# Abhipray/audio-codec

Hardware: AMD Instinct MI355X
Metric: audio channel-frames/s encode (48 kHz, 1024-line long blocks, 128 kb/s/ch) (higher is better)
Workload: dtype f64

## Files before the change

### audio-codec_amd/csrc/k_psy.hip

```cpp
#include "pacx_launch.h"
#include "mdct_dev.h"
#include "pcm_stage.h"
#include "wave_np_sum.h"
#include "quant_dev.h"


template <int DT>
__device__ __forceinline__ double hann_sample(const typename PcmStage<DT>::elem *raw, int i,
                                              const double *__restrict__ hw,
                                              const double *__restrict__ hw_pcm)
{
    if constexpr (DT == 0) {
        const int c = raw[i];
        return hw_pcm[i] * (double)(c == -32768 ? 0 : c);
    } else {
        return hw[i] * raw[i];
    }
}

#ifdef PACX_PSY_DEBUG
__device__ long long g_psy_dbg[16 * 16];
#define PSY_T(k) do { long long t_; asm volatile("s_waitcnt lgkmcnt(0)\n\ts_memtime %0\n\ts_waitcnt lgkmcnt(0)" : "=s"(t_) :: "memory"); \
                      if (dbg_on) dbg_acc[k] += t_ - dbg_last; dbg_last = t_; } while (0)
extern "C" int pacx_debug_read_psy(long long *out, int n)
// ... 526 lines not shown
        const int m = (64 - k) & 63;
        const cplx tm = c_mul(T.w128[m], po);
        cplx zm = c_add(pe, tm), zm5 = c_sub(pe, tm);
        if (k == 0) {
            zm5 = zk;
            zm = zk5;
        }
        ig[k] = pair_intensity(zk, zm5, T.w256[k], T.norm_short);
        ig[k + 64] = pair_intensity(zk5, zm, T.w256[k + 64], T.norm_short);
        if (k == 0)
            ig[128] = pair_intensity(zk, zk, T.w256[128], T.norm_short);
    }
    __syncthreads();

    int count = 0;
    for (int base = 0; base <= 128; base += 8) {
        const int i = base + r;
        bool pk = false;
        if (i >= 1 && i <= 128) {
            const double c = ig[i];
            pk = (c > ig[i - 1]) && (i == 128 || c > ig[i + 1]);
        }
        const unsigned m = (unsigned)((__builtin_amdgcn_ballot_w64(pk) >> (8 * g)) & 0xFFull);
        if (pk)
            pk_idx[g][count + __popc(m & ((1u << r) - 1u))] = (unsigned char)i;
        count += __popc(m);
    }
    if (r == 0) {
        pk_cnt[g] = count;
        n_peaks[cf * PACX_SUB + g] = count;
        n_kept_out[cf * PACX_SUB + g] = count;
    }
    __syncthreads();
    int start[PACX_SUB + 1];
    start[0] = 0;
#pragma unroll
    for (int q = 0; q < PACX_SUB; ++q)
        start[q + 1] = start[q] + pk_cnt[q];
    const int total = start[PACX_SUB];
    for (int t = lane; t < total; t += 64) {
        int q = 0;
#pragma unroll
        for (int u = 1; u < PACX_SUB; ++u)
            q += (t >= start[u]);
        const int p = t - start[q];
        const int i = pk_idx[q][p];
        const double *iq = inten + q * 130;
        peaks[cf * PACX_MAX_PEAKS + q * 64 + p] = make_peak(iq[i - 1], iq[i], i, T.fstep_short);
    }
}

#ifndef MASK_WAVES
#define MASK_WAVES 4
#endif
#ifndef MASK_OCC
#define MASK_OCC 3
#endif
#ifndef MASK_LDS_TABLES
#define MASK_LDS_TABLES 1
#endif
#ifndef MASK_OCC_PLAIN
#define MASK_OCC_PLAIN 4
#endif
#ifndef MASK_WG_PER_CU
#define MASK_WG_PER_CU 3
#endif
#ifndef MASK_WG_PER_CU_PLAIN
#define MASK_WG_PER_CU_PLAIN 4
#endif



__device__ __forceinline__ unsigned long long mask_key_of(double v)
{
    const unsigned long long u = (unsigned long long)__double_as_longlong(v);
    return (u >> 63) ? ~u : (u | 0x8000000000000000ull);
}
__device__ __forceinline__ double mask_value_of(unsigned long long k)
{
    const unsigned long long u = (k >> 63) ? (k & 0x7fffffffffffffffull) : ~k;
    return __longlong_as_double((long long)u);
}

#ifndef MASK_WAVES_PLAIN
#define MASK_WAVES_PLAIN 4
#endif
constexpr int mask_waves(int m, bool tail) { return (m == PACX_M_LONG && !tail) ? MASK_WAVES_PLAIN : MASK_WAVES; }

template <int M, bool TAIL>
__global__ __launch_bounds__(64 * mask_waves(M, TAIL), (M == PACX_M_LONG && !TAIL) ? MASK_OCC_PLAIN : MASK_OCC) void k_mask(PacxTables T, const uint8_t *__restrict__ flags,
                                                         int n_ch, long long n_units, int mixed,
                                                         const PacxPeak *__restrict__ peaks,
                                                         const int32_t *__restrict__ n_peaks,
                                                         const double *__restrict__ lines,
                                                         double *__restrict__ smr,
                                                         double *__restrict__ thr_out,
                                                         const int32_t *__restrict__ cf_list,
                                                         const int32_t *__restrict__ cf_count,
                                                         MaskTail tail)
{
    constexpr bool SHORT = (M == PACX_M_SHORT);
    constexpr int NW = mask_waves(M, TAIL);
    static_assert(!(TAIL && SHORT), "the fused tail is for long blocks");
    constexpr int PER = M / 64;
    constexpr bool BARK_LDS = (MASK_LDS_TABLES & 1) != 0, QUIET_LDS = (MASK_LDS_TABLES & 2) != 0;
    __shared__ __attribute__((aligned(16))) double bark_l[BARK_LDS ? M : 1];
    __shared__ __attribute__((aligned(16))) double quiet_l[QUIET_LDS ? M : 1];
    __shared__ __attribute__((aligned(16))) double chunk_c[PER][4];
    constexpr bool PAD = M / 64 == 16;
    constexpr int RJ = PAD ? PER / 2 : 0;
    constexpr int NH = PAD ? 2 : 1, HP = PER / NH;
    constexpr int MH = M / NH;
    constexpr int JSTR = PAD ? 72 : 64;
    __shared__ __attribute__((aligned(16))) double bufs[NW][MH + (PAD ? MH / 8 : 0)];
    __shared__ __attribute__((aligned(16))) double2 mk_zs_all[NW][64];
    __shared__ __attribute__((aligned(16))) double mk_u_all[NW][64];
    const int tid = threadIdx.x, lane = tid & 63, wv = tid >> 6;
    const double *__restrict__ bark_g = SHORT ? T.bark_short : T.bark_long;
    const double *__restrict__ quiet_g = SHORT ? T.thresh_short : T.thresh_long;
    for (int i = tid; i < M; i += 64 * NW) {
        if (BARK_LDS)
            bark_l[i] = bark_g[i];
        if (QUIET_LDS)
            quiet_l[i] = quiet_g[i];
    }
    __syncthreads();
    const double *bark_s = BARK_LDS ? (const double *)bark_l : bark_g;
    const double *quiet_s = QUIET_LDS ? (const double *)quiet_l : quiet_g;
    for (int j = wv; j < PER; j += NW) {
        double qm = quiet_s[64 * j + lane];
#pragma unroll
        for (int off = 32; off > 0; off >>= 1)
            qm = fmin(qm, __shfl_xor(qm, off, 64));
        if (lane == 0) {
            chunk_c[j][0] = bark_s[64 * j] - 0.5;
            chunk_c[j][1] = bark_s[64 * j + 63] + 0.5;
            chunk_c[j][2] = qm - 0.01;
        }
    }
    __syncthreads();

    double *buf = bufs[wv];
    const int sl = lane + (PAD ? lane >> 3 : 0);
    double2 *mk_zs = mk_zs_all[wv];
    double *mk_u = mk_u_all[wv];
    const int nb = SHORT ? T.nb_short : T.nb_long;
    const int32_t *__restrict__ lower = SHORT ? T.band_lower_short : T.band_lower_long;
    const int32_t *__restrict__ count = SHORT ? T.band_lines_short : T.band_lines_long;
    if (cf_list)
        n_units = SHORT ? (long long)(*cf_count) * PACX_SUB : (long long)(*cf_count);
#ifdef PACX_PSY_DEBUG
    const bool dbg_on = blockIdx.x == 5;
    long long dbg_acc[8] = {0, 0, 0, 0, 0, 0, 0, 0}, dbg_last = 0;
    unsigned long long st_pairs = 0, st_surv = 0, st_live = 0, st_batches = 0;
    PSY_T(7);
    dbg_acc[7] = 0;
#endif
    for (long long unit = (long long)blockIdx.x * NW + wv; unit < n_units;
         unit += (long long)gridDim.x * NW) {
        long long cf = SHORT ? unit / PACX_SUB : unit;
        const int sb = SHORT ? (int)(unit % PACX_SUB) : 0;
        if (cf_list) {
            cf = cf_list[cf];
        } else if (mixed) {
            const unsigned fl = flags ? flags[cf / n_ch] : 0u;
            if (SHORT != ((fl & 2u) != 0))
                continue;
        }
        const PacxPeak *__restrict__ pk = peaks + cf * PACX_MAX_PEAKS + sb * 64;
        const int np = n_peaks[cf * PACX_SUB + sb];
        const long long loff = cf * PACX_M_LONG + sb * PACX_M_SHORT;

        double rb[RJ ? RJ : 1];
#pragma unroll
        for (int j = 0; j < PER; ++j) {
            if (j < RJ)
                rb[j] = -INFINITY;
            else
                buf[sl + JSTR * (j - RJ)] = -INFINITY;
        }
        PacxPeak qn;
        qn.z = 0.0; qn.spl = -1000.0; qn.slope = 0.0;
        if (lane < np)
            qn = pk[lane];
        PSY_T(0);
        for (int pb = 0; pb < np; pb += 64) {
#ifdef PACX_PSY_DEBUG
            st_batches += 1;
#endif
            const PacxPeak q = qn;
            qn.z = 0.0; qn.spl = -1000.0; qn.slope = 0.0;
            if (pb + 64 + lane < np)
                qn = pk[pb + 64 + lane];
            const double lvl = q.spl - 16.0;
            const int n_in = min(64, np - pb);
            const double bz_lo = __hiloint2double(__builtin_amdgcn_readlane(__double2hiint(q.z), 0),
                                                  __builtin_amdgcn_readlane(__double2loint(q.z), 0));
            const double bz_hi = __hiloint2double(__builtin_amdgcn_readlane(__double2hiint(q.z), n_in - 1),
                                                  __builtin_amdgcn_readlane(__double2loint(q.z), n_in - 1));
            const double b_lvl = wave_max_upper(lvl);
            const double b_slope = wave_max_upper(q.slope);
            wave_lds_fence();
            mk_zs[lane] = make_double2(q.z, q.spl);
            mk_u[lane] = q.slope;
            wave_lds_fence();
#pragma unroll
            for (int j = 0; j < PER; ++j) {
                asm volatile("" ::: "memory");
                const double lo_edge = chunk_c[j][0], hi_edge = chunk_c[j][1], need = chunk_c[j][2];
                if (b_slope <= 0.0) {
                    double bb = 0.0;
                    if (bz_hi < lo_edge)
                        bb = b_slope * (lo_edge - bz_hi);
                    else if (bz_lo > hi_edge)
                        bb = -27.0 * (bz_lo - hi_edge);
                    if (b_lvl + bb <= need)
                        continue;
                }
                const double ub = q.slope * fmax(lo_edge - q.z, 0.0) + -27.0 * fmax(q.z - hi_edge, 0.0);
                const bool live = (q.slope > 0.0 && q.spl > -1000.0) || (lvl + ub > need);
                unsigned long long todo = __builtin_amdgcn_ballot_w64(live);
#ifdef PACX_PSY_DEBUG
                st_pairs += 1;
                st_surv += __popcll(todo);
                st_live += todo ? 1 : 0;
#endif
                if (!todo)
                    continue;
                const double zj = bark_s[lane + 64 * j];
                double bj;
                if (j < RJ)
                    bj = rb[j];
                else
                    bj = buf[sl + JSTR * (j - RJ)];
                while (todo) {
                    int bs[4];
#pragma unroll
                    for (int u = 0; u < 4; ++u) {
                        bs[u] = __builtin_ctzll(todo);
                        if (todo & (todo - 1))
                            todo &= todo - 1;
                        else if (u == 3)
                            todo = 0;
                    }
                    double2 zs[4];
                    double pus[4];
#pragma unroll
                    for (int u = 0; u < 4; ++u) {
                        zs[u] = mk_zs[bs[u]];
                        pus[u] = mk_u[bs[u]];
                    }
#pragma unroll
                    for (int u = 0; u < 4; ++u) {
                        const double pz = zs[u].x, ps = zs[u].y, pu = pus[u];
                        const double dz = zj - pz;
                        const double a = fmax(fabs(dz) - 0.5, 0.0);
                        const double gain = (dz < 0.0 ? -27.0 : pu) * a;
                        const double cand = (ps + gain) - 16.0;
                        asm("v_max_f64 %0, %1, %2" : "=v"(bj) : "v"(bj), "v"(cand));
                    }
                }
                if (j < RJ)
                    rb[j] = bj;
                else
                    buf[sl + JSTR * (j - RJ)] = bj;
            }
        }
        wave_lds_fence();
        PSY_T(1);
        double *__restrict__ out = smr ? smr + cf * T.band_stride + sb * T.nb_short : nullptr;
        unsigned long long *key = (unsigned long long *)mk_zs;
        key[lane] = 0ull;
#pragma unroll 1
        for (int h = NH - 1; h >= 0; --h) {
            if (RJ && h == 0) {
                wave_lds_fence();
#pragma unroll
                for (int j = 0; j < RJ; ++j)
                    buf[sl + JSTR * j] = rb[j];
                wave_lds_fence();
            }
            const int k0 = h * MH;
            double v_next = lines[loff + k0 + lane], q_next = quiet_s[k0 + lane];
#pragma unroll 1
            for (int j = 0; j < HP; ++j) {
                const int k = k0 + lane + 64 * j;
                const double v = v_next;
                double thr = q_next;
                if (j + 1 < HP) {
                    v_next = lines[loff + k + 64];
                    q_next = quiet_s[k + 64];
                }
                const double bst = buf[sl + JSTR * j];
                if (bst > -INFINITY)
                    thr = fmax(thr, mask_round_trip(bst));
                if (thr_out)
                    thr_out[loff + k] = thr;
                double it = (v * v) * 4.0;
                if (it == 0.0)
                    it = 1e-8;
                double spl = 96.0 + 10.0 * pacx_log10_pos(it + PACX_EPS);
                if (spl < -30.0)
                    spl = -30.0;
                buf[sl + JSTR * j] = spl - thr;
            }
            wave_lds_fence();
            int rl = lane;
            asm volatile("" : "+v"(rl));
            double v[HP];
            uint8_t bd[HP];
            if constexpr (SHORT) {
                const double2 t = *(const double2 *)(buf + 2 * rl);
                v[0] = t.x;
                v[1] = t.y;
                const uchar2 b2 = *(const uchar2 *)(T.line_band_short + 2 * rl);
                bd[0] = b2.x;
                bd[1] = b2.y;
            } else {
                static_assert(SHORT || HP == 8, "eight lines per lane and half");
                const uint2 b8 = *(const uint2 *)(T.line_band_long + k0 + 8 * rl);
                const unsigned w[2] = {b8.x, b8.y};
#pragma unroll
                for (int j = 0; j < HP; ++j) {
                    v[j] = buf[9 * rl + j];
                    bd[j] = (uint8_t)(w[j >> 2] >> (8 * (j & 3)));
                }
            }
            wave_lds_fence();
            int cur = bd[0];
            double mx = v[0];
#pragma unroll
            for (int j = 1; j < HP; ++j) {
                if (bd[j] != cur) {
                    atomicMax(&key[cur], mask_key_of(mx));
                    cur = bd[j];
                    mx = v[j];
                } else {
                    mx = fmax(mx, v[j]);
                }
            }
            atomicMax(&key[cur], mask_key_of(mx));
        }
        wave_lds_fence();
        PSY_T(2);
        const double s_l = mask_value_of(key[lane & 31]);
        if (out && lane < nb)
            out[lane] = s_l;
        {
            if constexpr (TAIL) {
                wave_lds_fence();
                int tl = lane;
                asm volatile("" : "+v"(tl));
                char *base = (char *)buf;
                unsigned *words = (unsigned *)base;
                double *cp = (double *)(base + PACX_PAYLOAD_STRIDE);
                unsigned long long *bmax = (unsigned long long *)(base + 2704);
                int *ba_s = (int *)(base + 2960), *sf_s = ba_s + PACX_MAX_BANDS;
                int *offs = sf_s + PACX_MAX_BANDS, *lower_s = offs + PACX_MAX_BANDS + 1;
                const int half = tl >> 5, l = tl & 31;
                const unsigned fl = flags ? flags[cf / n_ch] : 0u;
                const long long boff = cf * T.band_stride;
                const int32_t *__restrict__ n_lines = T.use_sbr ? T.band_lines_long_alloc : T.band_lines_long;
                const double budget = pacx_bit_budget(T.target_bps, PACX_M_LONG, 0, (fl & 5u) != 0, T.n_scale_bits,
                                                      T.n_mant_size_bits, nb, T.use_vq, T.use_sbr);
                int max_mant = 1 << T.n_mant_size_bits;
                if (max_mant > 16)
                    max_mant = 16;
                const bool has = half == 0 && l < nb;
                const int nl = has ? n_lines[l] : 0;
                int bits = 0, cap = 0;
                bitalloc_half(half == 0, has, has ? s_l : 0.0, nl, budget, max_mant, cp + 32 * half, half, l, bits, cap, T.guard != 0, T.nb_long);
                if (has) {
                    tail.bit_alloc[boff + l] = bits;
                    ba_s[l] = bits;
                }
                if (tl == nb && nb < PACX_MAX_BANDS)
                    ba_s[nb] = 0;
                if (cap && tail.status && tl == 0)
                    atomicOr(&tail.status[cf], ((cap & 1) ? 4u : 0u) | ((cap & 2) ? 16u : 0u));
                PSY_T(4);
                if (!T.use_vq) {
                    const int ov = tail.overall[cf * PACX_SUB];
                    const int k0 = 16 * tl;
                    int my_off = 0, a_mine = 0, end = 0;
                    if (tail.payload) {
                        for (int i = tl; i < PACX_PAYLOAD_WORDS; i += 64)
                            words[i] = 0u;
                        wave_lds_fence();
                        a_mine = (tl < nb) ? ba_s[tl] : 0;
                        const int width = (tl < nb) ? T.n_mant_size_bits + T.n_scale_bits + a_mine * count[tl] : 0;
                        int incl = width;
#pragma unroll
                        for (int off = 1; off < 32; off <<= 1) {
                            const int t = __shfl_up(incl, off, 64);
                            if (tl >= off)
                                incl += t;
                        }
                        my_off = 3 + T.n_scale_bits + incl - width;
                        end = __shfl(incl, nb - 1, 64) + 3 + T.n_scale_bits;
                        if (tl < nb) {
                            offs[tl] = my_off + T.n_mant_size_bits + T.n_scale_bits;
                            lower_s[tl] = lower[tl];
                        }
                        if (tl == 0) {
                            put_bits(words, 0, fl & 1u, 1);
                            put_bits(words, 1, (fl >> 1) & 1u, 1);
                            put_bits(words, 2, (fl >> 2) & 1u, 1);
                            put_bits(words, 3, (unsigned)ov, T.n_scale_bits);
                        }
                    }
                    double x[16];
                    uint8_t band[16];
                    long_scale_factors(T, lines + loff, (double)(1 << ov), bmax, ba_s, sf_s, tl, x, band);
                    if (tl < nb) {
                        tail.scale_factor[boff + tl] = sf_s[tl];
                        if (tail.payload) {
                            put_bits(words, my_off, (unsigned)(a_mine ? a_mine - 1 : 0), T.n_mant_size_bits);
                            put_bits(words, my_off + T.n_mant_size_bits, (unsigned)sf_s[tl], T.n_scale_bits);
                        }
                    }
                    PSY_T(5);
                    bool near = false;
#pragma unroll
                    for (int j4 = 0; j4 < 16; j4 += 4) {
                        int mq[4];
#pragma unroll
                        for (int u = 0; u < 4; ++u) {
                            const int j = j4 + u;
                            const int b = band[j];
                            const int a = ba_s[b];
                            mq[u] = a ? pacx_mantissa(x[j], sf_s[b], T.n_scale_bits, a) : 0;
                            if (T.guard)
                                near = near || pacx_quant_guard(fabs(x[j]), (1 << T.n_scale_bits) - 1 + a, PACX_GUARD_LINE_ERR);
                            if (tail.payload && a)
                                put_bits(words, offs[b] + (k0 + j - lower_s[b]) * a, (unsigned)mq[u], a);
                        }
                        if (tail.mantissa)
                            *(int4 *)(tail.mantissa + loff + k0 + j4) = make_int4(mq[0], mq[1], mq[2], mq[3]);
                    }
                    if (tail.status && __builtin_amdgcn_ballot_w64(near) && tl == 0)
                        atomicOr(&tail.status[cf], 16u);
                    if (tail.payload) {
                        wave_lds_fence();
                        const int nbytes = ((end - 3) + 4 + 7) >> 3;
                        unsigned *dst = (unsigned *)(tail.payload + cf * (long long)tail.payload_stride);
                        for (int i = tl; i < (nbytes + 3) / 4; i += 64)
                            dst[i] = __builtin_bswap32(words[i]);
                        if (tl == 0)
                            tail.n_bytes[cf] = nbytes;
                    }
                    PSY_T(6);
                }
            }
        }
        wave_lds_fence();
        PSY_T(3);
    }
#ifdef PACX_PSY_DEBUG
    if (dbg_on && lane == 0 && M == PACX_M_LONG)
        for (int k = 0; k < 8; ++k)
            g_psy_dbg[wv * 16 + k] = dbg_acc[k];
    if (lane == 0 && M == PACX_M_LONG) {
        atomicAdd((unsigned long long *)&g_psy_dbg[160], st_pairs);
        atomicAdd((unsigned long long *)&g_psy_dbg[161], st_surv);
        atomicAdd((unsigned long long *)&g_psy_dbg[162], st_live);
        atomicAdd((unsigned long long *)&g_psy_dbg[163], st_batches);
    }
#endif
}

#define SMRG_THREADS 256
__global__ __launch_bounds__(SMRG_THREADS) void k_smr_generic(long long n_blocks, int n, int nb,
                                                             const double *__restrict__ data,
                                                             const double *__restrict__ lines,
                                                             const double *__restrict__ hann,
                                                             const double *__restrict__ tw_cos,
                                                             const double *__restrict__ tw_sin, double norm,
                                                             double fstep, const double *__restrict__ bark,
                                                             const double *__restrict__ quiet,
                                                             const int32_t *__restrict__ band_lower,
                                                             const int32_t *__restrict__ band_count,
                                                             double *__restrict__ smr, double *__restrict__ thr_out,
                                                             int32_t *__restrict__ n_peaks_out)
{
    extern __shared__ __attribute__((aligned(16))) unsigned char smrg_lds[];
    const int half = n / 2, n_bins = half + 1, max_pk = half / 2 + 1;
    double *w = (double *)smrg_lds;
    double *inten = w + n;
    PacxPeak *pk = (PacxPeak *)(inten + n_bins + (n_bins & 1));
    __shared__ int n_pk;
    const int tid = threadIdx.x;
    const long long blk = blockIdx.x;
    if (blk >= n_blocks)
        return;
    const double *x = data + blk * n;
    for (int i = tid; i < n; i += SMRG_THREADS)
        w[i] = hann[i] * x[i];
    if (tid == 0)
        n_pk = 0;
    __syncthreads();
    for (int k = tid; k < n_bins; k += SMRG_THREADS) {
        double re = 0.0, im = 0.0;
        int m = 0;
        for (int i = 0; i < n; ++i) {
            re += w[i] * tw_cos[m];
            im -= w[i] * tw_sin[m];
            m += k;
            if (m >= n)
                m -= n;
        }
        const double a = sqrt(re * re + im * im);
        inten[k] = norm * (a * a);
    }
    __syncthreads();
    for (int i = 1 + tid; i < n_bins; i += SMRG_THREADS) {
        const double c = inten[i];
        if (c > inten[i - 1] && (i == n_bins - 1 || c > inten[i + 1])) {
            const int at = atomicAdd(&n_pk, 1);
            if (at < max_pk)
                pk[at] = make_peak(inten[i - 1], c, i, fstep);
        }
    }
    __syncthreads();
    const int np = n_pk < max_pk ? n_pk : max_pk;
    if (tid == 0 && n_peaks_out)
        n_peaks_out[blk] = np;
    const double *ln = lines + blk * half;
    for (int k = tid; k < half; k += SMRG_THREADS) {
        const double zj = bark[k];
        double best = -INFINITY;
        for (int p = 0; p < np; ++p) {
            const double dz = zj - pk[p].z;
            const double a = fmax(fabs(dz) - 0.5, 0.0);
            const double gain = (dz < 0.0 ? -27.0 : pk[p].slope) * a;
            best = fmax(best, (pk[p].spl + gain) - 16.0);
        }
        double thr = quiet[k];
        if (best > -INFINITY)
            thr = fmax(thr, mask_round_trip(best));
        if (thr_out)
            thr_out[blk * half + k] = thr;
        const double v = ln[k];
        double it = (v * v) * 4.0;
        if (it == 0.0)
            it = 1e-8;
        double spl = 96.0 + 10.0 * pacx_log10_pos(it + PACX_EPS);
        if (spl < -30.0)
            spl = -30.0;
        w[k] = spl - thr;
// ... 109 lines not shown
```

### audio-codec_amd/csrc/pacx_api.hip

```cpp
#include <hip/hip_runtime.h>

#include <math.h>
#include <stdio.h>
#include <stdlib.h>
#include <string.h>

#include <cmath>
#include <string>
#include <vector>

#include "../../include/pacx.h"
#include "body_index.h"
#include "pacx_launch.h"
#include "pvq_dev.h"
#include "pacx_vq_tables.h"
#include "pacx_tables_gen.h"

using namespace pacx_k;

struct PacxOverrides {
    int split_short;
    int fuse_tail;
    int fuse_front;
    int vq_fuse_alloc;
    int vq_frame;
    int vq_bfs;
    int vq_dec_frame;
};

#define PACX_FUSE_FRONT_DEFAULT 1

static int env_override(const char *name, int lo, int hi)
{
    const char *e = getenv(name);
    if (!e || !*e)
        return -1;
    char *end;
    const long v = strtol(e, &end, 10);
    return (*end || v < lo || v > hi) ? -1 : (int)v;
}

static PacxOverrides read_overrides(void)
{
    PacxOverrides o;
    o.split_short = env_override("PACX_SPLIT_SHORT", 0, 0);
    o.fuse_tail = env_override("PACX_FUSE_TAIL", 0, 1);
    o.fuse_front = env_override("PACX_FUSE_FRONT", 0, 1);
    o.vq_fuse_alloc = env_override("PACX_VQ_FUSE_ALLOC", 0, 1);
    o.vq_frame = env_override("PACX_VQ_FRAME", 0, 0);
    o.vq_bfs = env_override("PACX_VQ_BFS", 0, 1 << 20);
    o.vq_dec_frame = env_override("PACX_VQ_DEC_FRAME", 0, 0);
    return o;
}

struct pacx_handle {
    int device;
    int n_cu;
    PacxOverrides force;
    PacxTables T;
    std::vector<void *> owned;
    long long ws_cf;
    double *ws_lines;
    double *ws_smr;
    PacxPeak *ws_peaks;
    int32_t *ws_npeaks;
    int32_t *ws_nkept;
    int32_t *ws_overall;
    long long *ws_chunks;
    long long *ws_offs;
    int32_t *ws_lists;
    long long ws_blocks_cf;
    double *ws_blocks;
    int fork_side;
    hipStream_t side_stream;
    hipEvent_t ev_fork, ev_join;
    hipStream_t short_stream;
    hipStream_t spare_stream;
    hipEvent_t ev_short_done, ev_lists;
    std::vector<char> vq_view;
    std::vector<char> vqdec_view;
    int tables_exact;
    long long ws_mant_cf;
    int32_t *ws_mant;
    long long ws_dec_cf;
    double *ws_dec_lines;
    uint8_t *ws_dec_sbr;
    uint32_t *ws_dec_status;
    double *ws_sbr_mean;
    long long ws_vq_cf;
    unsigned *ws_unit_words;
    int32_t *ws_unit_bits;
    long long ws_index_bytes;
    char *ws_index;
    long long ws_thr_cf;
    double *ws_thr;
    uint32_t *ws_rate_status;
    long long ws_solve_n;
    char *ws_solve;
    long long *ws_seg;
    long long seg_host_n;
    long long *seg_host;
    hipEvent_t ev_seg;
    std::string err;
};

static thread_local std::string g_create_err;

static int fail(pacx_handle *h, int code, const std::string &msg)
{
    if (h)
        h->err = msg;
    else
        g_create_err = msg;
    return code;
}

#define HIP_TRY(h, call)                                                               \
    do {                                                                               \
        hipError_t e_ = (call);                                                        \
        if (e_ != hipSuccess)                                                          \
            return fail(h, PACX_E_HIP, std::string(#call) + ": " + hipGetErrorString(e_)); \
    } while (0)

static void drain_internal(pacx_handle *h);
#define HIP_TRY_FORKED(h, call)                                                        \
    do {                                                                               \
        hipError_t e_ = (call);                                                        \
        if (e_ != hipSuccess) {                                                        \
            drain_internal(h);                                                         \
            return fail(h, PACX_E_HIP, std::string(#call) + ": " + hipGetErrorString(e_)); \
        }                                                                              \
// ... 258 lines not shown
        TRY(upload(h, hsp.data(), hsp.size(), &T.hann_short_pcm));
    }

    {
        std::vector<double2> t;
        t = unit_circle(512, 8, 1, 8192);  TRY(upload(h, t.data(), t.size(), &T.tw_long));
        t = unit_circle(64, 8, 1, 1024);   TRY(upload(h, t.data(), t.size(), &T.tw_short));
        t = unit_circle(512, 2, 0, 512);   TRY(upload(h, t.data(), t.size(), &T.w512));
        t = unit_circle(512, 2, 0, 1024);
        for (int k = 1; k < 256; ++k)
            t[512 - k] = make_double2(-t[k].x, t[k].y);
        t[256].x = 0.0;
        TRY(upload(h, t.data(), t.size(), &T.w1024));
        t = unit_circle(1025, 2, 0, 2048);
        for (int k = 0; k <= 512; ++k)
            t[k + 512] = make_double2(t[k].y, -t[k].x);
        TRY(upload(h, t.data(), t.size(), &T.w2048));
        t = unit_circle(64, 2, 0, 128);    TRY(upload(h, t.data(), t.size(), &T.w128));
        t = unit_circle(129, 2, 0, 256);   TRY(upload(h, t.data(), t.size(), &T.w256));
    }

    {
        std::vector<double> bl(ML), tl(ML), bs(MS), ts(MS);
        const int ri = gen_rate_index(cfg->sample_rate);
        const double *g_bl = ri >= 0 ? (const double *)PACX_GEN_BARK_LONG + (size_t)ri * ML : nullptr;
        const double *g_tl = ri >= 0 ? (const double *)PACX_GEN_THRESH_LONG + (size_t)ri * ML : nullptr;
        const double *g_bs = ri >= 0 ? (const double *)PACX_GEN_BARK_SHORT + (size_t)ri * MS : nullptr;
        const double *g_ts = ri >= 0 ? (const double *)PACX_GEN_THRESH_SHORT + (size_t)ri * MS : nullptr;
        if (ri < 0 && (!cfg->bark_long || !cfg->thresh_long || !cfg->bark_short || !cfg->thresh_short))
            h->tables_exact = 0;
        for (int k = 0; k < ML; ++k) {
            const double f = (sr / (2 * ML)) * (k + 0.5);
            bl[k] = cfg->bark_long ? cfg->bark_long[k] : (g_bl ? g_bl[k] : pacx_bark(f));
            tl[k] = cfg->thresh_long ? cfg->thresh_long[k] : (g_tl ? g_tl[k] : pacx_thresh_quiet(f));
        }
        for (int k = 0; k < MS; ++k) {
            const double f = (sr / (2 * MS)) * (k + 0.5);
            bs[k] = cfg->bark_short ? cfg->bark_short[k] : (g_bs ? g_bs[k] : pacx_bark(f));
            ts[k] = cfg->thresh_short ? cfg->thresh_short[k] : (g_ts ? g_ts[k] : pacx_thresh_quiet(f));
        }
        TRY(upload(h, bl.data(), bl.size(), &T.bark_long));
        TRY(upload(h, tl.data(), tl.size(), &T.thresh_long));
        TRY(upload(h, bs.data(), bs.size(), &T.bark_short));
        TRY(upload(h, ts.data(), ts.size(), &T.thresh_short));
    }
    auto hanning_norm = [](int n) {
        long double acc = 0;
        for (int i = 0; i < n; ++i) {
            const long double w = 0.5L - 0.5L * cosl(2.0L * 3.14159265358979323846264338327950288L * i / (n - 1));
            acc += w * w;
        }
        return (double)(4.0L / ((long double)n * n * (acc / n)));
    };
    (void)hanning_norm;
    T.norm_long = cfg->fft_norm_long != 0.0 ? cfg->fft_norm_long : ((const double *)PACX_GEN_FFT_NORM)[0];
    T.norm_short = cfg->fft_norm_short != 0.0 ? cfg->fft_norm_short : ((const double *)PACX_GEN_FFT_NORM)[1];
    T.fstep_long = cfg->fft_freq_step_long != 0.0 ? cfg->fft_freq_step_long : 1.0 / (NL * (1.0 / sr));
    T.fstep_short = cfg->fft_freq_step_short != 0.0 ? cfg->fft_freq_step_short : 1.0 / (NS * (1.0 / sr));

    {
        std::vector<double> bb(NL / 2 + 1);
        for (int i = 0; i <= NL / 2; ++i)
            bb[i] = pacx_bark((double)i * T.fstep_long);
        TRY(upload(h, bb.data(), bb.size(), &T.bark_bin_long));
    }
    T.nb_long = cfg->n_bands_long;
    T.nb_short = cfg->n_bands_short;
    int covered_long = ML, covered_short = MS;
    TRY(build_bands(h, cfg->band_lines_long, T.nb_long, ML, &T.band_lower_long, &T.band_lines_long,
                    &T.line_band_long, &covered_long));
    TRY(build_bands(h, cfg->band_lines_short, T.nb_short, MS, &T.band_lower_short, &T.band_lines_short,
                    &T.line_band_short, &covered_short));
    if (covered_short < MS && T.nb_short >= 8) {
        g_create_err = "pacx_create: at most 7 short bands when they do not cover every line";
        pacx_destroy(h);
        return PACX_E_UNSUPPORTED;
    }
    T.band_stride = T.nb_long > PACX_SUB * T.nb_short ? T.nb_long : PACX_SUB * T.nb_short;
    T.n_scale_bits = cfg->n_scale_bits;
    T.n_mant_size_bits = cfg->n_mant_size_bits;
    T.target_bps = cfg->target_bits_per_sample;

    T.guard = cfg->guard ? 1 : 0;
    T.use_vq = cfg->use_vq ? 1 : 0;
    T.use_sbr = cfg->use_sbr ? 1 : 0;
    T.first_omitted = T.nb_long;
    T.band_lines_long_alloc = T.band_lines_long;
    if (T.use_sbr) {
        std::vector<int32_t> alloc_lines(cfg->band_lines_long, cfg->band_lines_long + T.nb_long);
        const int cut = (covered_long - 1) / 2;
        int at = 0;
        for (int b = 0; b < T.nb_long; ++b) {
            if (at >= cut) {
                if (T.first_omitted == T.nb_long)
                    T.first_omitted = b;
                alloc_lines[b] = 1;
            }
            at += cfg->band_lines_long[b];
        }
        if (T.nb_long - T.first_omitted > PACX_SUB) {
            g_create_err = "pacx_create: more than 8 SBR-omitted bands";
            pacx_destroy(h);
            return PACX_E_UNSUPPORTED;
        }
        TRY(upload(h, alloc_lines.data(), alloc_lines.size(), &T.band_lines_long_alloc));
    }
    PvqTables tab;
    memset(&tab, 0, sizeof(tab));
    tab.l_max = 1;
    const double *d_lt = nullptr;
    if (T.use_vq) {
        int l_max = 1;
        for (int b = 0; b < T.nb_long; ++b)
            l_max = cfg->band_lines_long[b] > l_max ? cfg->band_lines_long[b] : l_max;
        for (int b = 0; b < T.nb_short; ++b)
            l_max = cfg->band_lines_short[b] > l_max ? cfg->band_lines_short[b] : l_max;
        tab.l_max = l_max;
        PacxVqHostTables vt;
        pacx_vq_build(l_max, cfg->half_log2 ? cfg->half_log2 : (const double *)PACX_GEN_HALF_LOG2, &vt);
        if (vt.n_tab.empty()) {
            vt.n_tab.push_back(0);
            vt.p_tab.push_back(0);
        }
        TRY(upload(h, vt.n_tab.data(), vt.n_tab.size(), &tab.n_tab));
        TRY(upload(h, vt.p_tab.data(), vt.p_tab.size(), &tab.p_tab));
        TRY(upload(h, vt.row_off.data(), vt.row_off.size(), &tab.row_off));
        TRY(upload(h, vt.k_of.data(), vt.k_of.size(), &tab.k_of));
        TRY(upload(h, vt.w_of.data(), vt.w_of.size(), &tab.w_of));
        TRY(upload(h, vt.half_log2.data(), vt.half_log2.size(), &tab.half_log2));
        h->vq_view.resize(pacx_vq_view_size());
        std::vector<int32_t> sizes_long(cfg->band_lines_long, cfg->band_lines_long + T.nb_long);
        for (int b = T.first_omitted; b < T.nb_long; ++b)
            sizes_long[b] = 1;
        std::vector<double> lt((1u << PACX_VQ_THETA_TABLE_BITS) - 1, 0.0);
        memcpy(lt.data(), cfg->vq_log2_tan ? cfg->vq_log2_tan : (const double *)PACX_GEN_VQ_LOG2_TAN,
               sizeof(double) * lt.size());
        static_assert(sizeof(PACX_GEN_VQ_LOG2_TAN) / 8 == (1u << PACX_VQ_THETA_TABLE_BITS) - 1, "log2-tan table");
        TRY(upload(h, lt.data(), lt.size(), &d_lt));
        pacx_vq_view_fill(h->vq_view.data(), tab, cfg->log_mu1 != 0.0 ? cfg->log_mu1 : ((const double *)PACX_GEN_LOG_MU1)[0],
                          d_lt, sizes_long.data(), T.nb_long, cfg->band_lines_short, T.nb_short);
    }
    if (T.use_vq || T.use_sbr) {
        const int gr = cfg->sbr_gauss ? cfg->sbr_gauss_radius : 800;
        if (gr < 1 || gr > 4096) {
            g_create_err = "pacx_create: sbr_gauss_radius out of range";
            pacx_destroy(h);
            return PACX_E_ARG;
        }
        std::vector<double> gw(2 * gr + 1), lf(ML);
        static_assert(sizeof(PACX_GEN_SBR_GAUSS) / 8 == 2 * 800 + 1, "gaussian weights");
        memcpy(gw.data(), cfg->sbr_gauss ? cfg->sbr_gauss : (const double *)PACX_GEN_SBR_GAUSS,
               sizeof(double) * gw.size());
        for (int k = 0; k < ML; ++k)
            lf[k] = cfg->line_freq_long ? cfg->line_freq_long[k] : (k + 0.5) * (sr / (2 * ML));
        const double *d_gw, *d_lf;
        TRY(upload(h, gw.data(), gw.size(), &d_gw));
        TRY(upload(h, lf.data(), lf.size(), &d_lf));
        h->vqdec_view.resize(pacx_vqdec_view_size());
        pacx_vqdec_view_fill(h->vqdec_view.data(), tab, d_lt, d_gw, gr, d_lf, cfg->band_lines_long, T.nb_long,
                             cfg->band_lines_short, T.nb_short);
    }
#undef TRY
    *out = h;
    return PACX_OK;
}

// ... 1408 lines not shown
```

### audio-codec_amd/csrc/pacx_dev.h

```cpp
#ifndef PACX_DEV_H
#define PACX_DEV_H

#include <hip/hip_runtime.h>
#include <stdint.h>

#include "pacx_exact.h"

#define PACX_N_LONG 2048
#define PACX_M_LONG 1024
#define PACX_N_SHORT 256
#define PACX_M_SHORT 128
#define PACX_SUB 8
#define PACX_SHORT_FIRST 448
#define PACX_MAX_PEAKS 512
#define PACX_PAYLOAD_STRIDE 2192
#define PACX_PAYLOAD_WORDS (PACX_PAYLOAD_STRIDE / 4)

struct PacxTables {
    const double *win_long;
    const double *win_short;
    const double *hann_long;
    const double *hann_short;
    const double *ones;
    const double *kbd_long;
    const double *kbd_short;
    const double *hann_long_pcm;
    const double *hann_short_pcm;
    const double2 *tw_long;
    const double2 *tw_short;
    const double2 *w512;
    const double2 *w1024;
    const double2 *w2048;
    const double2 *w128;
    const double2 *w256;
    const double *bark_long, *thresh_long;
    const double *bark_short, *thresh_short;
    const double *bark_bin_long;
    const int32_t *band_lower_long, *band_lines_long;
    const int32_t *band_lower_short, *band_lines_short;
    const uint8_t *line_band_long;
    const uint8_t *line_band_short;
    double norm_long, norm_short;
    double fstep_long, fstep_short;
    double target_bps;
    int nb_long, nb_short;
    int n_scale_bits, n_mant_size_bits;
    int band_stride;
    int use_vq, use_sbr;
    int first_omitted;
    const int32_t *band_lines_long_alloc;
    int guard;
};

struct PacxPcmView {
    const void *base;
    long long frame_stride, ch_stride, samp_stride;
    int n_ch;
};

struct __attribute__((aligned(8))) PacxPeak {
    double z;
    double spl;
    double slope;
};

#define PACX_PART_LONG  (1 << 4)
#define PACX_PART_SHORT (2 << 4)

struct MaskTail {
    const int32_t *overall;
    int32_t *bit_alloc;
    int32_t *scale_factor;
    int32_t *mantissa;
    uint32_t *status;
    uint8_t *payload;
    int32_t *n_bytes;
    int payload_stride;
};

__device__ __forceinline__ unsigned pacx_xcd_block(unsigned b, unsigned n_blocks)
{
    return (n_blocks & 7u) ? b : (b & 7u) * (n_blocks >> 3) + (b >> 3);
}
__device__ __forceinline__ long long pacx_xcd_frame(unsigned b, unsigned n_blocks, long long n_cf)
{
    if ((n_cf & 2047) != 0 || n_blocks != (unsigned)n_cf)
        return b;
    const unsigned idx = b >> 3;
    return (long long)(idx >> 8) * 2048 + (b & 7u) * 256 + (idx & 255u);
}

struct PacxIndexWs {
    long long n_seg, n_groups;
    size_t tab;
    size_t gtab;
    size_t gentry;
    size_t gbase;
    size_t entry;
    size_t base;
    size_t fin;
};

#endif
```

### audio-codec_amd/csrc/pacx_exact.h

```cpp
#ifndef PACX_EXACT_H
#define PACX_EXACT_H

#include <math.h>
#include <stdint.h>
#include <string.h>

#if defined(__HIPCC__)
#define PACX_HD __host__ __device__ __forceinline__
#else
#define PACX_HD static inline
#endif

#define PACX_MAX_BANDS 32
#define PACX_ALLOC_MAX_PASSES 200
#define PACX_DB_PER_BIT 6.2
#define PACX_EPS 2.220446049250313e-16
#define PACX_VQ_SPLIT_BITS 32
#define PACX_VQ_THETA_TABLE_BITS 12

PACX_HD double pacx_pcm16_to_f64(int c)
{
    const int neg = c < 0;
    const int mag = (neg ? -c : c) & 32767;
    const double n = (double)(2 * mag);
// ... 359 lines not shown
    rc = fma(fma(-d, rc, 1.0), rc, rc);
    double sq = f * rc;
    sq = fma(fma(-d, sq, f), rc, sq);
    const double z = sq * sq, w = z * z;
#if defined(__HIP_DEVICE_COMPILE__)
#define PACX_FMA_SC(r, a, b, c) asm("v_fma_f64 %0, %1, %2, %3" : "=v"(r) : "v"(a), "v"(b), "s"(c))
#else
#define PACX_FMA_SC(r, a, b, c) (r) = fma((a), (b), (c))
#endif
    double h1, h2;
    PACX_FMA_SC(h1, w, Lg6, Lg4);
    PACX_FMA_SC(h1, w, h1, Lg2);
    PACX_FMA_SC(h2, w, Lg7, Lg5);
    PACX_FMA_SC(h2, w, h2, Lg3);
    PACX_FMA_SC(h2, w, h2, Lg1);
#undef PACX_FMA_SC
    const double t1 = w * h1;
    const double t2 = z * h2;
    const double r = sq * (hfsq + (t2 + t1));
    double hi = f - hfsq;
    memcpy(&bits, &hi, 8);
    bits &= 0xFFFFFFFF00000000ull;
    memcpy(&hi, &bits, 8);
    const double lo = ((f - hi) - hfsq) + r;
    double val_hi = hi * ivln10hi;
    const double y2 = dk * log10_2hi;
    double val_lo = fma(dk, log10_2lo, fma(lo + hi, ivln10lo, lo * ivln10hi));
    const double wv = y2 + val_hi;
    val_lo += (y2 - wv) + val_hi;
    return val_lo + wv;
}

PACX_HD double pacx_spl_array(double intensity)
{
    if (intensity == 0.0)
        intensity = 1e-8;
    double spl = 96.0 + 10.0 * log10(fabs(intensity) + PACX_EPS);
    if (spl < -30.0)
        spl = -30.0;
    return spl;
}

PACX_HD double pacx_exp2_lean(double y)
{
    const double n = rint(y), f = y - n;
    const double c1 = 6.931471805599453094e-01, c2 = 2.402265069591007123e-01, c3 = 5.550410866482157995e-02,
                 c4 = 9.618129107628477162e-03, c5 = 1.333355814642844343e-03, c6 = 1.540353039338160995e-04,
                 c7 = 1.525273380405984028e-05, c8 = 1.321548679014430949e-06, c9 = 1.017808600923969973e-07,
                 c10 = 7.054911620801123330e-09;
#if defined(__HIP_DEVICE_COMPILE__)
#define PACX_FMA_SC(r, a, b, c) asm("v_fma_f64 %0, %1, %2, %3" : "=v"(r) : "v"(a), "v"(b), "s"(c))
#else
#define PACX_FMA_SC(r, a, b, c) (r) = fma((a), (b), (c))
#endif
    double p;
    PACX_FMA_SC(p, f, c10, c9);
    PACX_FMA_SC(p, f, p, c8);
    PACX_FMA_SC(p, f, p, c7);
    PACX_FMA_SC(p, f, p, c6);
    PACX_FMA_SC(p, f, p, c5);
    PACX_FMA_SC(p, f, p, c4);
    PACX_FMA_SC(p, f, p, c3);
    PACX_FMA_SC(p, f, p, c2);
    PACX_FMA_SC(p, f, p, c1);
#undef PACX_FMA_SC
    p = fma(f, p, 1.0);
    int e = (int)n;
    return ldexp(p, e);
}

PACX_HD double pacx_spl_of_intensity_of(double x)
{
    double y = (96.0 - x) * 0.33219280948873623;
    if (y > 1000.0)
        y = 1000.0;
    const double t = PACX_EPS * pacx_exp2_lean(y);
    if (!(t < 1e-3))
        return -30.0;
    const double p = t * (1.0 + t * (-0.5 + t * (1.0 / 3.0 + t * (-0.25 + t * 0.2))));
    const double r = x + 4.3429448190325182765 * p;
    return r < -30.0 ? -30.0 : r;
}

PACX_HD double pacx_spl_scalar(double intensity)
{
    if (intensity == 0.0)
        return -30.0;
    double spl = 96.0 + 10.0 * log10(fabs(intensity) + PACX_EPS);
    if (spl < -30.0)
        spl = -30.0;
    return spl;
}

PACX_HD double pacx_bark(double f)
{
    const double t = f / 7500.0;
    return 13.0 * atan(0.76 * f / 1000.0) + 3.5 * atan(t * t);
}

PACX_HD double pacx_thresh_quiet(double f)
{
    if (f < 10.0)
        f = 10.0;
    const double k = f / 1000.0;
    const double d = k - 3.3;
    return 3.64 * pow(k, -0.8) - 6.5 * exp(-0.6 * (d * d)) + 0.001 * (k * k * k * k);
}

PACX_HD int pacx_window_kind(unsigned flags)
{
    const int last_t = flags & 1u, cur_t = (flags >> 1) & 1u, next_t = (flags >> 2) & 1u;
    if (cur_t) return 0;
    if (last_t && next_t) return 3;
    if (last_t) return 2;
    if (next_t) return 1;
    return 0;
}

#endif
```

### audio-codec_amd/engine.py

```python
import ctypes

import numpy as np
import torch

from . import _lib, tables
from .psychoac import ScaleFactorBands, AssignMDCTLinesFromFreqLimits

N_LONG, N_SHORT = 1024, 128


def _ptr(t):
    return ctypes.c_void_p(t.data_ptr()) if t is not None else None


class PcmView:

    def __init__(self, tensor, n_channels, n_frames, frame_stride, channel_stride,
                 sample_stride=1):
        if tensor.dtype == torch.int16:
            dt = _lib.PCM_I16
        elif tensor.dtype == torch.float64:
            dt = _lib.PCM_F64
        else:
            raise TypeError("PCM must be int16 codes or float64 signed fractions")
# ... 602 lines not shown
    def _elem(self, name, x, *ints):
        x = x.contiguous()
        out = self._empty(x.shape, torch.int64)
        self._call(name, ctypes.c_int64(x.numel()), _ptr(x), *[int(i) for i in ints], _ptr(out),
                   self._stream())
        return out

    def quantize_uniform(self, x, n_bits):
        return self._elem("pacx_quantize_uniform", x, n_bits)

    def scale_factor(self, x, n_scale_bits, n_mant_bits):
        return self._elem("pacx_scale_factor", x, n_scale_bits, n_mant_bits)

    def mantissa(self, x, scale, n_scale_bits, n_mant_bits):
        return self._elem("pacx_mantissa", x, scale, n_scale_bits, n_mant_bits)

    def mantissa_fp(self, x, scale, n_scale_bits, n_mant_bits):
        return self._elem("pacx_mantissa_fp", x, scale, n_scale_bits, n_mant_bits)

    def _delem(self, name, codes, *ints):
        codes = codes.contiguous()
        assert codes.dtype == torch.int64
        out = self._empty(codes.shape, torch.float64)
        self._call(name, ctypes.c_int64(codes.numel()), _ptr(codes), *[int(i) for i in ints], _ptr(out),
                   self._stream())
        return out

    def dequantize_uniform(self, codes, n_bits):
        return self._delem("pacx_dequantize_uniform", codes, n_bits)

    def dequantize(self, mant, scale, n_scale_bits, n_mant_bits):
        return self._delem("pacx_dequantize", mant, scale, n_scale_bits, n_mant_bits)

    def dequantize_fp(self, mant, scale, n_scale_bits, n_mant_bits):
        return self._delem("pacx_dequantize_fp", mant, scale, n_scale_bits, n_mant_bits)

    def imdct(self, lines, short=False):
        lines = lines.contiguous().view(-1, N_LONG)
        out = self._empty((lines.shape[0], 2 * N_LONG), torch.float64)
        self._call("pacx_imdct_batch", ctypes.c_int64(lines.shape[0]), _lib.MDCT_SHORT if short else 0, _ptr(lines),
                   _ptr(out), self._stream())
        return out

    def mdct_direct(self, x, a, b, inverse=False):
        n_in = (a + b) // 2 if inverse else a + b
        n_out = a + b if inverse else (a + b) // 2
        x = x.contiguous().view(-1, n_in)
        out = self._empty((x.shape[0], n_out), torch.float64)
        self._call("pacx_mdct_direct_batch", ctypes.c_int64(x.shape[0]), int(a), int(b), int(bool(inverse)), _ptr(x),
                   _ptr(out), self._stream())
        return out

    def transient_detect(self, blocks, thresh=4.5):
        blocks = blocks.contiguous()
        n, n_ch, ln = blocks.shape
        out = self._empty((n,), torch.uint8)
        self._call("pacx_transient_detect_f64", ctypes.c_int64(n), int(n_ch), int(ln), _ptr(blocks),
                   ctypes.c_double(float(thresh)), _ptr(out), self._stream())
        return out

    def bit_alloc_generic(self, budget, max_mant_bits, n_lines, smr):
        smr = smr.contiguous()
        n, nb = smr.shape
        nl = torch.as_tensor(np.asarray(n_lines, dtype=np.int32), device=self.device)
        bits = self._empty((n, nb), torch.int32)
        self._call("pacx_bitalloc_generic", ctypes.c_int64(n), int(nb), _ptr(nl), _ptr(budget.contiguous()),
                   int(max_mant_bits), _ptr(smr), _ptr(bits), self._stream())
        return bits


class EncoderPool:

    def __init__(self, n, *args, **kwargs):
        self.encs = [Encoder(*args, **kwargs) for _ in range(max(1, int(n)))]
        dev = self.encs[0].device
        self.streams = [torch.cuda.Stream(device=dev) for _ in self.encs]
        self.done = [torch.cuda.Event() for _ in self.encs]
        self._turn = 0
        self._gate = self._gate_stream = None
        self._used = [False] * len(self.encs)
        if len(self.encs) > 1:
            for e in self.encs:
                e.set_side_fork(True)

    def __len__(self):
        return len(self.encs)

    def next(self):
        k = self._turn
        self._turn = (k + 1) % len(self.encs)
        return k

    def slot(self, k):
        pool = self

        class _Slot:
            def __enter__(self_inner):
                self_inner.ctx = torch.cuda.stream(pool.streams[k])
                self_inner.ctx.__enter__()
                return pool.encs[k]

            def __exit__(self_inner, *exc):
                pool.done[k].record(pool.streams[k])
                pool._used[k] = True
                return self_inner.ctx.__exit__(*exc)
        return _Slot()

    def align(self, delay_us=None):
        if len(self.encs) < 2:
            return
        if delay_us is None:
            delay_us = float(os.environ.get("PACX_POOL_GATE_US", "100"))
        if delay_us <= 0 or not hasattr(torch.cuda, "_sleep"):
            return
        dev = self.encs[0].device
        if self._gate is None:
            self._gate_stream = torch.cuda.Stream(device=dev)
            self._gate = torch.cuda.Event()
            t0, t1 = torch.cuda.Event(enable_timing=True), torch.cuda.Event(enable_timing=True)
            with torch.cuda.stream(self._gate_stream):
                torch.cuda._sleep(100_000)
                t0.record()
                torch.cuda._sleep(2_000_000)
                t1.record()
            t1.synchronize()
            self._cycles_per_us = 2_000_000 / max(t0.elapsed_time(t1) * 1e3, 1.0)
        with torch.cuda.stream(self._gate_stream):
            for k in range(len(self.encs)):
                if self._used[k]:
                    self._gate_stream.wait_event(self.done[k])
            torch.cuda._sleep(int(delay_us * self._cycles_per_us))
            self._gate.record(self._gate_stream)
        for s in self.streams:
            s.wait_event(self._gate)

    def wait(self, k, stream=None):
        (stream or torch.cuda.current_stream(self.encs[0].device)).wait_event(self.done[k])

    def synchronize(self):
        for s in self.streams:
            s.synchronize()

    def close(self):
        for e in self.encs:
            e.close()
```

Before: 52.57 million.

## Screen mask lines with cheap float log before exact per-band SMR max

Adds a screening pass to the long-block mask kernel. It computes an approximate per-line SMR using a float log2 and a lower-bound threshold, takes a per-band approximate max, and keeps only lines within a small delta of that max. Only those candidates, up to 64 per half, are evaluated with the exact double-precision SPL and mask round trip, and it falls back to the full path on overflow. This is meant to avoid the exact per-line log and threshold conversion for most of the 1024 lines, at the cost of extra ballots, LDS atomics and a rigorously bounded approximation window. It also moves the pool gate calibration into the constructor so it is no longer done on the first align call.

```diff
diff --git a/audio-codec_amd/csrc/k_psy.hip b/audio-codec_amd/csrc/k_psy.hip
--- a/audio-codec_amd/csrc/k_psy.hip
+++ b/audio-codec_amd/csrc/k_psy.hip
@@ -632,6 +632,7 @@
     return __longlong_as_double((long long)u);
 }
 
+#define MASK_CAND 64
 #ifndef MASK_WAVES_PLAIN
 #define MASK_WAVES_PLAIN 4
 #endif
@@ -658,6 +659,7 @@
     __shared__ __attribute__((aligned(16))) double quiet_l[QUIET_LDS ? M : 1];
     __shared__ __attribute__((aligned(16))) double chunk_c[PER][4];
     constexpr bool PAD = M / 64 == 16;
+    constexpr bool SCREEN = PAD && !TAIL;
     constexpr int RJ = PAD ? PER / 2 : 0;
     constexpr int NH = PAD ? 2 : 1, HP = PER / NH;
     constexpr int MH = M / NH;
@@ -703,6 +705,7 @@
     const bool dbg_on = blockIdx.x == 5;
     long long dbg_acc[8] = {0, 0, 0, 0, 0, 0, 0, 0}, dbg_last = 0;
     unsigned long long st_pairs = 0, st_surv = 0, st_live = 0, st_batches = 0;
+    unsigned long long st_halves = 0, st_cand = 0, st_over = 0;
     PSY_T(7);
     dbg_acc[7] = 0;
 #endif
@@ -821,8 +824,105 @@
         double *__restrict__ out = smr ? smr + cf * T.band_stride + sb * T.nb_short : nullptr;
         unsigned long long *key = (unsigned long long *)mk_zs;
         key[lane] = 0ull;
+        const bool screen = SCREEN && T.mask_lines != 0 && !thr_out;
+        unsigned long long *xkey = screen ? key + 32 : key;
+        auto load_runs = [&](int k0, int rl, double (&v)[HP], uint8_t (&bd)[HP]) {
+            if constexpr (SHORT) {
+                const double2 t = *(const double2 *)(buf + 2 * rl);
+                v[0] = t.x;
+                v[1] = t.y;
+                const uchar2 b2 = *(const uchar2 *)(T.line_band_short + 2 * rl);
+                bd[0] = b2.x;
+                bd[1] = b2.y;
+            } else {
+                static_assert(SHORT || HP == 8, "eight lines per lane and half");
+                const uint2 b8 = *(const uint2 *)(T.line_band_long + k0 + 8 * rl);
+                const unsigned w[2] = {b8.x, b8.y};
+#pragma unroll
+                for (int j = 0; j < HP; ++j) {
+                    v[j] = buf[9 * rl + j];
+                    bd[j] = (uint8_t)(w[j >> 2] >> (8 * (j & 3)));
+                }
+            }
+        };
+        auto post_runs = [&](unsigned long long *keys, const double (&v)[HP], const uint8_t (&bd)[HP]) {
+            int cur = bd[0];
+            double mx = v[0];
+#pragma unroll
+            for (int j = 1; j < HP; ++j) {
+                if (bd[j] != cur) {
+                    atomicMax(&keys[cur], mask_key_of(mx));
+                    cur = bd[j];
+                    mx = v[j];
+                } else {
+                    mx = fmax(mx, v[j]);
+                }
+            }
+            atomicMax(&keys[cur], mask_key_of(mx));
+        };
 #pragma unroll 1
         for (int h = NH - 1; h >= 0; --h) {
+            const int k0 = h * MH;
+            if constexpr (SCREEN) {
+                if (screen) {
+                    const double delta = T.mask_lines == 2 ? INFINITY : PACX_SCREEN_DELTA;
+                    if (h == 0) {
+                        wave_lds_fence();
+#pragma unroll
+                        for (int j = 0; j < RJ; ++j)
+                            buf[sl + JSTR * j] = rb[j];
+                    }
+                    wave_lds_fence();
+                    int rl = lane;
+                    asm volatile("" : "+v"(rl));
+                    double a[HP];
+                    uint8_t bd[HP];
+                    const double2 *__restrict__ vp = (const double2 *)(lines + loff + k0 + 8 * rl);
+                    const double2 *__restrict__ qp = (const double2 *)(quiet_s + k0 + 8 * rl);
+                    const uint2 b8 = *(const uint2 *)(T.line_band_long + k0 + 8 * rl);
+                    const unsigned w[2] = {b8.x, b8.y};
+#pragma unroll
+                    for (int j = 0; j < HP; j += 2) {
+                        const double2 tv = vp[j >> 1], tq = qp[j >> 1];
+                        a[j] = pacx_screen_a(tv.x, buf[9 * rl + j], tq.x);
+                        a[j + 1] = pacx_screen_a(tv.y, buf[9 * rl + j + 1], tq.y);
+                    }
+#pragma unroll
+                    for (int j = 0; j < HP; ++j)
+                        bd[j] = (uint8_t)(w[j >> 2] >> (8 * (j & 3)));
+                    post_runs(key, a, bd);
+                    wave_lds_fence();
+                    int *cl_k = (int *)mk_u;
+                    double lim = 0.0;
+                    int n_cand = 0;
+#pragma unroll
+                    for (int j = 0; j < HP; ++j) {
+                        if (j == 0 || bd[j] != bd[j - 1])
+                            lim = mask_value_of(key[bd[j]]) - delta;
+                        const bool c = a[j] >= lim;
+                        const unsigned long long m = __builtin_amdgcn_ballot_w64(c);
+                        const int pos = n_cand + (int)__builtin_amdgcn_mbcnt_hi((unsigned)(m >> 32),
+                                                                               __builtin_amdgcn_mbcnt_lo((unsigned)m, 0u));
+                        if (c && pos < MASK_CAND)
+                            cl_k[pos] = (8 * rl + j) | ((int)bd[j] << 16);
+                        n_cand += __popcll(m);
+                    }
+                    wave_lds_fence();
+#ifdef PACX_PSY_DEBUG
+                    st_halves += 1;
+                    st_cand += n_cand;
+                    st_over += n_cand > MASK_CAND ? 1 : 0;
+#endif
+                    if (n_cand <= MASK_CAND) {
+                        if (lane < n_cand) {
+                            const int kb = cl_k[lane], kk = kb & 0xffff, k = k0 + kk;
+                            const double e = pacx_mask_line_exact(lines[loff + k], buf[kk + (kk >> 3)], quiet_s[k]);
+                            atomicMax(&xkey[kb >> 16], mask_key_of(e));
+                        }
+                        continue;
+                    }
+                }
+            }
             if (RJ && h == 0) {
                 wave_lds_fence();
 #pragma unroll
@@ -830,7 +930,6 @@
                     buf[sl + JSTR * j] = rb[j];
                 wave_lds_fence();
             }
-            const int k0 = h * MH;
             double v_next = lines[loff + k0 + lane], q_next = quiet_s[k0 + lane];
 #pragma unroll 1
             for (int j = 0; j < HP; ++j) {
@@ -859,41 +958,13 @@
             asm volatile("" : "+v"(rl));
             double v[HP];
             uint8_t bd[HP];
-            if constexpr (SHORT) {
-                const double2 t = *(const double2 *)(buf + 2 * rl);
-                v[0] = t.x;
-                v[1] = t.y;
-                const uchar2 b2 = *(const uchar2 *)(T.line_band_short + 2 * rl);
-                bd[0] = b2.x;
-                bd[1] = b2.y;
-            } else {
-                static_assert(SHORT || HP == 8, "eight lines per lane and half");
-                const uint2 b8 = *(const uint2 *)(T.line_band_long + k0 + 8 * rl);
-                const unsigned w[2] = {b8.x, b8.y};
-#pragma unroll
-                for (int j = 0; j < HP; ++j) {
-                    v[j] = buf[9 * rl + j];
-                    bd[j] = (uint8_t)(w[j >> 2] >> (8 * (j & 3)));
-                }
-            }
+            load_runs(k0, rl, v, bd);
             wave_lds_fence();
-            int cur = bd[0];
-            double mx = v[0];
-#pragma unroll
-            for (int j = 1; j < HP; ++j) {
-                if (bd[j] != cur) {
-                    atomicMax(&key[cur], mask_key_of(mx));
-                    cur = bd[j];
-                    mx = v[j];
-                } else {
-                    mx = fmax(mx, v[j]);
-                }
-            }
-            atomicMax(&key[cur], mask_key_of(mx));
+            post_runs(xkey, v, bd);
         }
         wave_lds_fence();
         PSY_T(2);
-        const double s_l = mask_value_of(key[lane & 31]);
+        const double s_l = mask_value_of(xkey[lane & 31]);
         if (out && lane < nb)
             out[lane] = s_l;
         {
@@ -1015,6 +1086,9 @@
         atomicAdd((unsigned long long *)&g_psy_dbg[161], st_surv);
         atomicAdd((unsigned long long *)&g_psy_dbg[162], st_live);
         atomicAdd((unsigned long long *)&g_psy_dbg[163], st_batches);
+        atomicAdd((unsigned long long *)&g_psy_dbg[164], st_halves);
+        atomicAdd((unsigned long long *)&g_psy_dbg[165], st_cand);
+        atomicAdd((unsigned long long *)&g_psy_dbg[166], st_over);
     }
 #endif
 }
diff --git a/audio-codec_amd/csrc/pacx_api.hip b/audio-codec_amd/csrc/pacx_api.hip
--- a/audio-codec_amd/csrc/pacx_api.hip
+++ b/audio-codec_amd/csrc/pacx_api.hip
@@ -23,12 +23,14 @@
     int fuse_tail;
     int fuse_front;
     int vq_fuse_alloc;
+    int mask_lines;
     int vq_frame;
     int vq_bfs;
     int vq_dec_frame;
 };
 
 #define PACX_FUSE_FRONT_DEFAULT 1
+#define PACX_MASK_LINES_DEFAULT 1
 
 static int env_override(const char *name, int lo, int hi)
 {
@@ -47,6 +49,7 @@
     o.fuse_tail = env_override("PACX_FUSE_TAIL", 0, 1);
     o.fuse_front = env_override("PACX_FUSE_FRONT", 0, 1);
     o.vq_fuse_alloc = env_override("PACX_VQ_FUSE_ALLOC", 0, 1);
+    o.mask_lines = env_override("PACX_MASK_LINES", 0, 2);
     o.vq_frame = env_override("PACX_VQ_FRAME", 0, 0);
     o.vq_bfs = env_override("PACX_VQ_BFS", 0, 1 << 20);
     o.vq_dec_frame = env_override("PACX_VQ_DEC_FRAME", 0, 0);
@@ -471,6 +474,7 @@
     T.target_bps = cfg->target_bits_per_sample;
 
     T.guard = cfg->guard ? 1 : 0;
+    T.mask_lines = h->force.mask_lines >= 0 ? h->force.mask_lines : PACX_MASK_LINES_DEFAULT;
     T.use_vq = cfg->use_vq ? 1 : 0;
     T.use_sbr = cfg->use_sbr ? 1 : 0;
     T.first_omitted = T.nb_long;
diff --git a/audio-codec_amd/csrc/pacx_dev.h b/audio-codec_amd/csrc/pacx_dev.h
--- a/audio-codec_amd/csrc/pacx_dev.h
+++ b/audio-codec_amd/csrc/pacx_dev.h
@@ -50,6 +50,7 @@
     int first_omitted;
     const int32_t *band_lines_long_alloc;
     int guard;
+    int mask_lines;
 };
 
 struct PacxPcmView {
diff --git a/audio-codec_amd/csrc/pacx_exact.h b/audio-codec_amd/csrc/pacx_exact.h
--- a/audio-codec_amd/csrc/pacx_exact.h
+++ b/audio-codec_amd/csrc/pacx_exact.h
@@ -465,6 +465,53 @@
     return r < -30.0 ? -30.0 : r;
 }
 
+#define PACX_SCREEN_RT_MAX 4.35e-3
+#define PACX_SCREEN_E_LOG 1e-4
+#define PACX_SCREEN_DELTA 0.01
+#if defined(__cplusplus)
+static_assert(PACX_SCREEN_DELTA >= 2.0 * (PACX_SCREEN_RT_MAX + 2.0 * PACX_SCREEN_E_LOG),
+              "the candidate window keeps a factor two over the derived bound");
+#endif
+
+PACX_HD double pacx_screen_thr_lo(double bst, double quiet)
+{
+    const double t = fmax(quiet, fmax(bst, -30.0));
+    return bst > -INFINITY ? t : quiet;
+}
+
+PACX_HD double pacx_screen_spl(double x)
+{
+#if defined(__HIP_DEVICE_COMPILE__)
+    const float l2 = __builtin_amdgcn_logf((float)x);
+#else
+    const float l2 = log2f((float)x);
+#endif
+    const float s = fmaf(l2, 3.01029995663981195f, 96.0f);
+    return (double)fmaxf(s, -30.0f);
+}
+
+PACX_HD double pacx_screen_a(double v, double bst, double quiet)
+{
+    double it = (v * v) * 4.0;
+    if (it == 0.0)
+        it = 1e-8;
+    return pacx_screen_spl(it + PACX_EPS) - pacx_screen_thr_lo(bst, quiet);
+}
+
+PACX_HD double pacx_mask_line_exact(double v, double bst, double quiet)
+{
+    double thr = quiet;
+    if (bst > -INFINITY)
+        thr = fmax(thr, pacx_spl_of_intensity_of(bst));
+    double it = (v * v) * 4.0;
+    if (it == 0.0)
+        it = 1e-8;
+    double spl = 96.0 + 10.0 * pacx_log10_pos(it + PACX_EPS);
+    if (spl < -30.0)
+        spl = -30.0;
+    return spl - thr;
+}
+
 PACX_HD double pacx_spl_scalar(double intensity)
 {
     if (intensity == 0.0)
diff --git a/audio-codec_amd/engine.py b/audio-codec_amd/engine.py
--- a/audio-codec_amd/engine.py
+++ b/audio-codec_amd/engine.py
@@ -708,6 +708,20 @@
         if len(self.encs) > 1:
             for e in self.encs:
                 e.set_side_fork(True)
+            if hasattr(torch.cuda, "_sleep"):
+                self._calibrate_gate()
+
+    def _calibrate_gate(self):
+        self._gate_stream = torch.cuda.Stream(device=self.encs[0].device)
+        self._gate = torch.cuda.Event()
+        t0, t1 = torch.cuda.Event(enable_timing=True), torch.cuda.Event(enable_timing=True)
+        with torch.cuda.stream(self._gate_stream):
+            torch.cuda._sleep(100_000)
+            t0.record()
+            torch.cuda._sleep(2_000_000)
+            t1.record()
+        t1.synchronize()
+        self._cycles_per_us = 2_000_000 / max(t0.elapsed_time(t1) * 1e3, 1.0)
 
     def __len__(self):
         return len(self.encs)
@@ -739,18 +753,8 @@
             delay_us = float(os.environ.get("PACX_POOL_GATE_US", "100"))
         if delay_us <= 0 or not hasattr(torch.cuda, "_sleep"):
             return
-        dev = self.encs[0].device
         if self._gate is None:
-            self._gate_stream = torch.cuda.Stream(device=dev)
-            self._gate = torch.cuda.Event()
-            t0, t1 = torch.cuda.Event(enable_timing=True), torch.cuda.Event(enable_timing=True)
-            with torch.cuda.stream(self._gate_stream):
-                torch.cuda._sleep(100_000)
-                t0.record()
-                torch.cuda._sleep(2_000_000)
-                t1.record()
-            t1.synchronize()
-            self._cycles_per_us = 2_000_000 / max(t0.elapsed_time(t1) * 1e3, 1.0)
+            self._calibrate_gate()
         with torch.cuda.stream(self._gate_stream):
             for k in range(len(self.encs)):
                 if self._used[k]:
```

New measurement: 55.97 million, median of 6. 6.5% higher.
